# lambdaclass/simpleworks

Hardware: AMD Instinct MI355X
Metric: Marlin prove() constraints/sec at 2^20 R1CS; G1 MSM points/sec (higher is better)
Workload: dtype u32 limbs (384-bit Montgomery Fq for G1, 256-bit Fr); 1 GPU; marlin_prove: synthetic R1CS, 2^20 constraints = variables = non-zeros per matrix (|H| = |K| = 2^20), SRS + proving key device resident; per_gpu_units=1048576, multi_gpu=replicas (one proof per rank)

## Files before the change

simpleworks_amd/_lib.py:

```python
import ctypes
import json
import os

import numpy as np

_HERE = os.path.dirname(os.path.abspath(__file__))
LIB_PATH = os.environ.get("SWM_LIB_PATH") or os.path.join(_HERE, "libswmarlin.so")

_u64p = ctypes.POINTER(ctypes.c_uint64)
_u32p = ctypes.POINTER(ctypes.c_uint32)
_vp = ctypes.c_void_p
_sz = ctypes.c_size_t
_int = ctypes.c_int

ABI = {
    "swm_version": (_int, []),
    "swm_strerror": (ctypes.c_char_p, [_int]),
    "swm_init": (_int, [_int, ctypes.POINTER(_vp)]),
    "swm_destroy": (None, [_vp]),
    "swm_last_error": (ctypes.c_char_p, [_vp]),
    "swm_set_stream": (_int, [_vp, _vp]),
    "swm_set_msm_sharding": (_int, [_vp, ctypes.c_uint, ctypes.c_uint, _vp, _vp]),
    "swm_rccl_unique_id": (_int, [ctypes.c_void_p]),
    "swm_rccl_init": (_int, [_vp, ctypes.c_void_p, ctypes.c_uint, ctypes.c_uint]),
# ... 1192 lines not shown
        jac = np.zeros((n, 18), dtype=np.uint64) if backmap else None
        self._check(self.lib.swm_selftest_p28(self.h, self.P28_OPS[op], _p64(a) if a is not None else None,
                                              _p64(b) if b is not None else None, _p32(flags) if flags is not None else None,
                                              _p64(out), _p64(jac) if backmap else None, _p32(status), n), "swm_selftest_p28")
        return out, status[:n], jac

    def _poly(self, op, data, n, m, z, pieces, out):
        zz = np.ascontiguousarray(z if z is not None else np.zeros(4), dtype=np.uint64).reshape(4)
        pc = np.ascontiguousarray(pieces if pieces is not None else np.zeros(2), dtype=np.uint64).reshape(-1)
        self._check(self.lib.swm_selftest_poly(self.h, op, data.ctypes.data, n, m, _p64(zz), _p64(pc), pc.size // 2,
                                               out.ctypes.data if out is not None else None), "swm_selftest_poly")

    def selftest_suffix_recurrence(self, a_mont, m, z_mont):
        a = np.ascontiguousarray(a_mont, dtype=np.uint64).reshape(-1, 4).copy()
        self._poly(0, a, a.shape[0], m, z_mont, None, None)
        return a

    def selftest_div_linear(self, p_mont, z_mont):
        p = np.ascontiguousarray(p_mont, dtype=np.uint64).reshape(-1, 4)
        out = np.zeros_like(p)
        self._poly(1, p, p.shape[0], 0, z_mont, None, out)
        return out

    def selftest_poly_eval(self, p_mont, z_mont):
        p = np.ascontiguousarray(p_mont, dtype=np.uint64).reshape(-1, 4)
        out = np.zeros(4, dtype=np.uint64)
        self._poly(2, p, p.shape[0], 0, z_mont, None, out)
        return out

    def selftest_poly_eval_many(self, buf_mont, pieces, z_mont):
        buf = np.ascontiguousarray(buf_mont, dtype=np.uint64).reshape(-1, 4)
        pc = np.asarray(pieces, dtype=np.uint64).reshape(-1, 2)
        out = np.zeros((pc.shape[0], 4), dtype=np.uint64)
        self._poly(3, buf, buf.shape[0], 0, z_mont, pc, out)
        return out

    def selftest_ntt_from(self, src_mont, log_n, inverse=False, coset=False):
        src = np.ascontiguousarray(src_mont, dtype=np.uint64).reshape(-1, 4).copy()
        out = np.zeros((1 << log_n, 4), dtype=np.uint64)
        self._poly(4 + int(bool(inverse)) + 2 * int(bool(coset)), src, src.shape[0], log_n, None, None, out)
        return out, src

    def selftest_ntt_cosets(self, coeffs_mont, log_n, ks):
        src = np.ascontiguousarray(coeffs_mont, dtype=np.uint64).reshape(-1, 4).copy()
        kk = np.ascontiguousarray(ks, dtype=np.uint64).reshape(-1)
        out = np.zeros((kk.size << log_n, 4), dtype=np.uint64)
# ... 56 lines not shown
```

simpleworks_amd/csrc/devops.cuh:

```cuda
#pragma once
#include <chrono>
#include <exception>
#include <functional>
#include <utility>
#include <atomic>
#include "context.h"
#include "ff.cuh"
#include "fill.cuh"
#include "fr29.cuh"
#include "host/chacha.h"
#include "host/marlin_types.h"

namespace swm {

int ntt_run(swm_ctx* ctx, void* d_data, unsigned log_n, int inverse, int coset);
int ntt_run_from(swm_ctx* ctx, void* d_data, unsigned log_n, int inverse, int coset, const void* first_src, size_t src_len);
int ntt_cosets_fwd(swm_ctx* ctx, const void* coeffs, size_t len, unsigned log_n, const unsigned* ks, unsigned ncos, void* out);
int ntt_cosets_inv(swm_ctx* ctx, void* data, unsigned log_n, unsigned ncos);
int ntt_sharded_run(swm_ctx* ctx, void* d_local, unsigned log_n, int inverse, int blocks_in);
struct SpmvPlanHost {
    uint64_t nnz = 0, max_row = 0;
    std::vector<uint32_t> chunks, lrows;
};
struct SpmvPlan {
// ... 51 lines not shown
            }
        }
        p = nullptr;
    }
    void zero() { hip_check(ctx, zero_fill_async(p, n * sizeof(T), ctx->stream), "memset"); }
    void upload(const T* h, size_t count) {
        hip_check(ctx, hipMemcpyAsync(p, h, count * sizeof(T), hipMemcpyHostToDevice, ctx->stream), "h2d");
        hip_check(ctx, hipStreamSynchronize(ctx->stream), "sync");
    }
    std::vector<T> download(size_t off, size_t count) const {
        std::vector<T> h(count);
        hip_check(ctx, hipMemcpyAsync(h.data(), p + off, count * sizeof(T), hipMemcpyDeviceToHost, ctx->stream), "d2h");
        hip_check(ctx, hipStreamSynchronize(ctx->stream), "sync");
        return h;
    }
};
typedef DBuf<Fr> DVec;

inline DVec dv_zeros(swm_ctx* ctx, size_t n) {
    DVec v(ctx, n);
    v.zero();
    return v;
}
inline DVec dv_copy_padded(swm_ctx* ctx, const Fr* src, size_t len, size_t n) {
    DVec v(ctx, n);
    if (len > n) len = n;
    if (len) hip_check(ctx, hipMemcpyAsync(v.p, src, len * sizeof(Fr), hipMemcpyDeviceToDevice, ctx->stream), "d2d");
    if (n > len) hip_check(ctx, zero_fill_async(v.p + len, (n - len) * sizeof(Fr), ctx->stream), "memset");
    return v;
}

static __global__ void swm_proof_begin() {}

template <class F>
static __global__ void __launch_bounds__(256) ew_kernel(size_t n, F f) {
    SWM_LIGHT_KERNEL();
    for (size_t i = blockIdx.x * (size_t)blockDim.x + threadIdx.x; i < n; i += (size_t)gridDim.x * blockDim.x) f(i);
}
template <class F>
inline void ew(swm_ctx* ctx, const char* name, size_t n, F f) {
    if (n == 0) return;
    unsigned grid = (unsigned)std::min<size_t>((n + 255) / 256, 256 * 32);
    prof_begin(ctx, name);
    hipLaunchKernelGGL(ew_kernel<F>, dim3(grid), dim3(256), 0, ctx->stream, n, f);
    prof_end(ctx);
    hip_check(ctx, hipGetLastError(), name);
}

struct PowTable {
    const Fr* lo;
    const Fr* hi;
    __device__ __forceinline__ Fr at(uint64_t e) const {
// ... 109 lines not shown
static __global__ void __launch_bounds__(256) rec_tile_total29(const Fr* __restrict__ a, size_t n, RecConsts rc,
                                                               const Fr* __restrict__ zlow ,
                                                               Fr* __restrict__ totals) {
    SWM_LIGHT_KERNEL();
    __shared__ Fr sm[256];
    const size_t base = (size_t)blockIdx.x * RT_TILE;
    const unsigned t = threadIdx.x;
    const Fr29 z256 = fr29_unpack(rc.z256);
    Fr29 acc = fr29_zero();
#pragma unroll 1
    for (int j = RT_PER - 1; j >= 0; j--) {
        size_t k = base + (size_t)j * 256 + t;
        acc = fr29_mul_fenced(acc, z256);
        if (k < n) acc = fr29_add(acc, fr29_unpack(a[k]));
    }
    sm[t] = fr29_pack(fr29_canonical(fr29_mul_fenced(acc, fr29_unpack(zlow[t])), true));
    __syncthreads();
    for (unsigned s = 128; s > 0; s >>= 1) {
        if (t < s) sm[t] = fp_add(sm[t], sm[t + s]);
        __syncthreads();
    }
    if (t == 0) totals[blockIdx.x] = fp_mul(sm[0], rc.zpow[0]);
}
static __global__ void __launch_bounds__(256) rec_tile_scan29(Fr* __restrict__ a, size_t n, RecConsts rc,
                                                              const Fr* __restrict__ tile_true , size_t ntiles) {
    SWM_LIGHT_KERNEL();
    extern __shared__ __align__(16) unsigned char smem_raw[];
    Fr* tile = reinterpret_cast<Fr*>(smem_raw);
    Fr* hs = tile + RT_TILE + 256;
    const size_t b = blockIdx.x, base = b * RT_TILE;
    const unsigned t = threadIdx.x;
#pragma unroll
    for (int j = 0; j < RT_PER; j++) {
        unsigned e = j * 256 + t;
        size_t k = base + e;
        tile[rt_pad(e)] = k < n ? a[k] : fp_zero<Fr>();
    }
    __syncthreads();
    Fr29 loc[RT_PER];
    {
        const Fr29 z1 = fr29_unpack(rc.zpow[1]);
        Fr29 acc = fr29_zero();
#pragma unroll
        for (int i = RT_PER - 1; i >= 0; i--) {
            acc = fr29_add(fr29_unpack(tile[rt_pad(t * RT_PER + i)]), fr29_mul_fenced(acc, z1));
            loc[i] = acc;
        }
        hs[t] = fr29_pack(fr29_below_2r(acc));
    }
    if (t == 0) hs[256] = b + 1 < ntiles ? tile_true[b + 1] : fp_zero<Fr>();
    __syncthreads();
#pragma unroll 1
    for (int k = 0; k < 9; k++) {
        unsigned d = 1u << k;
        Fr v = hs[t];
        bool has = t + d <= 256;
        Fr o = has ? hs[t + d] : fp_zero<Fr>();
        __syncthreads();
        if (has) hs[t] = fr29_pack(fr29_below_2r(fr29_add(fr29_unpack(v), fr29_mul_fenced(fr29_unpack(o), fr29_unpack(rc.zstep[k])))));
        __syncthreads();
    }
    const Fr29 carry = fr29_unpack(hs[t + 1]);
#pragma unroll
    for (int i = 0; i < RT_PER; i++) {
        const Fr29 v = fr29_add(loc[i], fr29_mul_fenced(carry, fr29_unpack(rc.zpow[RT_PER - i])));
        tile[rt_pad(t * RT_PER + i)] = fr29_pack(fr29_cond_sub(fr29_cond_sub(fr29_cond_sub(fr29_normalize(v), Fr29Consts::P2), Fr29Consts::P2), Fr29Consts::P));
    }
    __syncthreads();
#pragma unroll
    for (int j = 0; j < RT_PER; j++) {
        unsigned e = j * 256 + t;
        size_t k = base + e;
        if (k < n) a[k] = tile[rt_pad(e)];
    }
}

inline void suffix_recurrence(swm_ctx* ctx, Fr* a, size_t n, size_t m, const Fr& z);
inline void suffix_recurrence_tiled(swm_ctx* ctx, Fr* a, size_t n, const Fr& z) {
    size_t ntiles = (n + RT_TILE - 1) / RT_TILE;
    RecConsts rc;
    rc.zpow[0] = fp_one<Fr>();
    for (int i = 1; i <= RT_PER; i++) rc.zpow[i] = fp_mul(rc.zpow[i - 1], z);
    rc.zstep[0] = rc.zpow[RT_PER];
    for (int k = 1; k < 9; k++) rc.zstep[k] = fp_sqr(rc.zstep[k - 1]);
    DVec zlow(ctx, 256), totals(ctx, ntiles);
    rc.z256 = dv_pow256(ctx, z, zlow.p);
    RecConsts rc29;
    const Fr two5 = fp_from_u64<Fr>(32);
    for (int i = 0; i <= RT_PER; i++) rc29.zpow[i] = fp_mul(rc.zpow[i], two5);
    for (int k = 0; k < 9; k++) rc29.zstep[k] = fp_mul(rc.zstep[k], two5);
    rc29.z256 = fp_mul(rc.z256, two5);
    prof_begin(ctx, "rec_tile_total");
    hipLaunchKernelGGL(rec_tile_total29, dim3((unsigned)ntiles), dim3(256), 0, ctx->stream, (const Fr*)a, n, rc29, (const Fr*)zlow.p, totals.p);
    prof_end(ctx);
    hip_check(ctx, hipGetLastError(), "rec_tile_total");
    Fr ztile = rc.z256;
    for (int i = 0; i < 3; i++) ztile = fp_sqr(ztile);
    static_assert(RT_TILE == 2048, "tile exponent");
    suffix_recurrence(ctx, totals.p, ntiles, 1, ztile);
    size_t lds = (size_t)(RT_TILE + 256 + 257) * sizeof(Fr);
    static std::atomic<bool> attr_set[64];
    if (!attr_set[ctx->device & 63].load(std::memory_order_acquire)) {
        hip_check(ctx, hipFuncSetAttribute((const void*)rec_tile_scan29, hipFuncAttributeMaxDynamicSharedMemorySize, (int)lds), "attr");
        attr_set[ctx->device & 63].store(true, std::memory_order_release);
    }
    prof_begin(ctx, "rec_tile_scan");
    hipLaunchKernelGGL(rec_tile_scan29, dim3((unsigned)ntiles), dim3(256), lds, ctx->stream, a, n, rc29, (const Fr*)totals.p, ntiles);
    prof_end(ctx);
    hip_check(ctx, hipGetLastError(), "rec_tile_scan");
}

inline void suffix_recurrence(swm_ctx* ctx, Fr* a, size_t n, size_t m, const Fr& z) {
    if (n == 0) return;
    if (m == 1 && n >= 4 * (size_t)RT_TILE) {
        suffix_recurrence_tiled(ctx, a, n, z);
        return;
    }
    size_t rows = (n + m - 1) / m;
    if (rows <= REC_T) {
        prof_begin(ctx, "rec_serial");
        hipLaunchKernelGGL(rec_serial, dim3((unsigned)((m + 63) / 64)), dim3(64), 0, ctx->stream, a, n, m, z);
        prof_end(ctx);
        hip_check(ctx, hipGetLastError(), "rec_serial");
        return;
    }
    size_t nblk = (rows + REC_T - 1) / REC_T;
    DVec head(ctx, nblk * m);
    unsigned grid = (unsigned)((nblk * m + 255) / 256);
    prof_begin(ctx, "rec_local");
    hipLaunchKernelGGL(rec_local, dim3(grid), dim3(256), 0, ctx->stream, a, n, m, z, head.p, nblk);
    prof_end(ctx);
    hip_check(ctx, hipGetLastError(), "rec_local");
    Fr zt = z;
    for (int i = 0; i < 4; i++) zt = fp_sqr(zt);
    static_assert(REC_T == 16, "zt exponent");
    suffix_recurrence(ctx, head.p, nblk * m, m, zt);
    prof_begin(ctx, "rec_fix");
    hipLaunchKernelGGL(rec_fix, dim3(grid), dim3(256), 0, ctx->stream, a, n, m, z, head.p, nblk);
    prof_end(ctx);
    hip_check(ctx, hipGetLastError(), "rec_fix");
}

struct DivResult {
    DVec work;
};
inline DivResult div_linear(swm_ctx* ctx, const Fr* p, size_t n, const Fr& x, size_t cap = 0) {
    DivResult r;
    r.work = dv_copy_padded(ctx, p, n, std::max<size_t>({n, cap, 1}));
    if (n == 0) r.work.zero();
    suffix_recurrence(ctx, r.work.p, n, 1, x);
    return r;
}

static constexpr int EVAL_PER = 16;
static constexpr int EVAL_TILE = 256 * EVAL_PER;
static __global__ void __launch_bounds__(256) eval_chunks(const Fr* __restrict__ c, size_t n, Fr x256, const Fr* __restrict__ xpow,
                                                          Fr* __restrict__ out) {
    SWM_LIGHT_KERNEL();
    __shared__ Fr sm[256];
    const size_t base = (size_t)blockIdx.x * EVAL_TILE;
    const unsigned t = threadIdx.x;
    Fr acc = fp_zero<Fr>();
#pragma unroll 1
    for (int j = EVAL_PER - 1; j >= 0; j--) {
        size_t k = base + (size_t)j * 256 + t;
        acc = fp_mul(acc, x256);
        if (k < n) acc = fp_add(acc, c[k]);
    }
    sm[t] = fp_mul(acc, xpow[t]);
    __syncthreads();
    for (unsigned s = 128; s > 0; s >>= 1) {
        if (t < s) sm[t] = fp_add(sm[t], sm[t + s]);
// ... 472 lines not shown
```

simpleworks_amd/csrc/marlin.hip:

```cpp
#include <stdlib.h>
#include <string.h>
#include <algorithm>
#include <chrono>
#include <functional>
#include <memory>
#include <type_traits>
#include "devops.cuh"
#include "g1.cuh"
#include "host/ahp.h"

#include "msm.h"
using namespace swm;

#define LAUNCHX(ctx, name, kernel, grid, block, shmem, ...)                         \
    do {                                                                            \
        prof_begin(ctx, name);                                                      \
        hipLaunchKernelGGL(kernel, grid, block, shmem, (ctx)->stream, __VA_ARGS__); \
        prof_end(ctx);                                                              \
        hip_check(ctx, hipGetLastError(), name);                                    \
    } while (0)

#include "host/pk_codec.h"
#include "host/host_handles.h"
struct swm_srs {
// ... 934 lines not shown
    return sp;
}
DVec shard_evals(swm_ctx* ctx, const ShardPlan& sp, const Fr* coeffs, size_t n, unsigned log) {
    const size_t len = ((size_t)1 << log) / sp.SG;
    DVec loc(ctx, len);
    Fr* out = loc.p;
    const size_t s_rank = sp.rank, s_world = sp.SG;
    ew(ctx, "shard_take_cyclic", len, [=] __device__(size_t j) {
        const size_t i = s_rank + s_world * j;
        out[j] = i < n ? coeffs[i] : fp_zero<Fr>();
    });
    rc_check(ctx, ntt_sharded_run(ctx, loc.p, log, 0, 0));
    return loc;
}
void shard_gather_cyclic(swm_ctx* ctx, const Fr* loc, size_t per, unsigned lg, Fr* dst, size_t n) {
    DVec all(ctx, per << lg);
    rc_check(ctx, shard_allgather_dev(ctx, loc, per * sizeof(Fr), all.p));
    const Fr* src = all.p;
    ew(ctx, "shard_interleave", n, [=] __device__(size_t i) { dst[i] = src[(i & (((size_t)1 << lg) - 1)) * per + (i >> lg)]; });
}
void add_rho_vh(swm_ctx* ctx, Fr* poly, uint64_t H, const Fr& rho) {
    ew(ctx, "add_rho_vh", 1, [=] __device__(size_t) {
        poly[0] = fp_sub(poly[0], rho);
        poly[H] = fp_add(poly[H], rho);
    });
}
void div_vh(swm_ctx* ctx, const Fr* q, size_t part, size_t total, Fr* h, Fr* g) {
    ew(ctx, "div_vh", 3 * part, [=] __device__(size_t j) {
        Fr acc = q[j + part];
        if (j + 2 * part < total) acc = fp_add(acc, q[j + 2 * part]);
        if (j + 3 * part < total) acc = fp_add(acc, q[j + 3 * part]);
        h[j] = acc;
        if (j < part) g[j] = fp_add(q[j], acc);
    });
}
void div_vk(swm_ctx* ctx, const Fr* q, size_t part, size_t total, Fr* h) {
    ew(ctx, "div_vk", 3 * part, [=] __device__(size_t j) {
        Fr acc = fp_zero<Fr>();
        for (uint64_t i = 1; j + i * part < total; i++) acc = fp_add(acc, q[j + i * part]);
        h[j] = acc;
    });
}
#ifndef SWM_OUTER_COSETS
#define SWM_OUTER_COSETS 1
#endif
static constexpr uint64_t OUTER_COSETS_MIN_H = 16;
struct Cosets3 {
// ... 29 lines not shown
};
struct CosetsMap {
    unsigned logD;
    __host__ __device__ size_t index(size_t p) const { return ((p & (((size_t)1 << logD) - 1)) << 2) + (p >> logD); }
    __host__ __device__ size_t position(size_t i) const { return ((i & 3) << logD) + (i >> 2); }
};
template <class F>
void with_product_map(const ShardPlan& sp, bool sharded, size_t loc, bool cosets, unsigned logD, F&& f) {
    if (sharded) f(BlocksMap{loc, loc / sp.SG, sp.rank});
    else if (cosets) f(CosetsMap{logD});
    else f(DenseMap{});
}
__device__ __forceinline__ Fr round2_outer_form(const Fr& eta_a, const Fr& eta_b, const Fr& eta_c, const Fr& ra, const Fr& a,
                                                const Fr& b, const Fr& z, const Fr& t) {
    const Fr summed = fp_add(fp_add(fp_mul(eta_c, fp_mul(a, b)), fp_mul(eta_a, a)), fp_mul(eta_b, b));
    return fp_sub(fp_mul(ra, summed), fp_mul(z, t));
}
struct IndexOnB {
    const Fr *ar, *ac, *arc, *av;
    const Fr *br, *bc, *brc, *bv;
    const Fr *cr, *cc, *crc, *cv;
};
struct Round3Challenges {
    Fr alpha, beta, ab, eta_a, eta_b, eta_c, vhab;
};
__device__ __forceinline__ Fr round3_a_minus_bf(const IndexOnB& x, const Round3Challenges& c, size_t i, const Fr& f) {
    Fr da = fp_add(fp_sub(fp_sub(c.ab, fp_mul(x.ar[i], c.alpha)), fp_mul(c.beta, x.ac[i])), x.arc[i]);
    Fr db = fp_add(fp_sub(fp_sub(c.ab, fp_mul(x.br[i], c.alpha)), fp_mul(c.beta, x.bc[i])), x.brc[i]);
    Fr dc = fp_add(fp_sub(fp_sub(c.ab, fp_mul(x.cr[i], c.alpha)), fp_mul(c.beta, x.cc[i])), x.crc[i]);
    Fr dbc = fp_mul(db, dc);
    Fr t = fp_add(fp_add(fp_mul(fp_mul(c.eta_a, x.av[i]), dbc), fp_mul(fp_mul(fp_mul(c.eta_b, x.bv[i]), da), dc)),
                  fp_mul(fp_mul(fp_mul(c.eta_c, x.cv[i]), da), db));
    Fr a_val = fp_mul(c.vhab, t);
    Fr b_val = fp_mul(da, dbc);
    return fp_sub(a_val, fp_mul(b_val, f));
}
struct ProveState {
    ChaChaRng& zk;
    PhaseTrace& tr;
    const ProveShape shape;
    const ShardPlan sp;
    const uint64_t H, K, X, Bsz, M;
    const unsigned logM;
    const size_t nvars, ninst;
    const size_t mask_len;
    const HDomain dh;
    const std::vector<Fr> public_input;
    FiatShamirRng fs;
    VerifierState st;
    Fr rho_w, rho_a, rho_b;
    int lane = 0;
    LPoly P_w, P_za, P_zb, P_mask, P_t, P_g1, P_h1, P_g2, P_h2;
    LPoly idx_polys[12];
    std::map<std::string, LPoly*> polys;
    CommitJob j1[4], j2[3], j3[2];
    std::vector<Commitment> comms1 = std::vector<Commitment>(4), comms2 = std::vector<Commitment>(3),
                            comms3 = std::vector<Commitment>(2);
    bool mask_late = false;
    unsigned mask_pieces = 1;
    AsyncMsm mask_part[2];
    bool ra_closed_form = false;
    bool cosets = false;
    LcSet lcs;
    DVec mask, z, za_evals, zb_evals, za_loc, zb_loc, x_poly, x_evals, w_poly, za_poly, zb_poly, e_za, e_zb, e_z;
    DVec r_alpha_evals, e_ra, t_poly, q1, h1, g1x, f, h2;

    ProveState(const swm_pk& pk, ChaChaRng& rng, PhaseTrace& t, ProveShape shp, const ShardPlan& plan)
        : zk(rng), tr(t), shape(std::move(shp)), sp(plan), H(pk.H), K(pk.K), X(pk.X), Bsz(pk.B), M(4 * pk.H),
          logM(pk.logH + 2), nvars(pk.info.num_variables), ninst(shape.inst.size()), mask_len(3 * pk.H), dh(pk.H),
          public_input(shape.inst.begin() + 1, shape.inst.end()) {
        fs_init(fs, pk.vk, public_input);
        for (int m = 0; m < 3; m++) {
            const DVec* v[4] = {&pk.ar[m].row, &pk.ar[m].col, &pk.ar[m].val, &pk.ar[m].row_col};
            for (int j = 0; j < 4; j++) {
                idx_polys[4 * m + j].p = v[j]->p;
                idx_polys[4 * m + j].n = K;
                polys[kIndexerPolys[4 * m + j]] = &idx_polys[4 * m + j];
            }
        }
        polys["w"] = &P_w; polys["z_a"] = &P_za; polys["z_b"] = &P_zb; polys["mask_poly"] = &P_mask;
        polys["t"] = &P_t; polys["g_1"] = &P_g1; polys["h_1"] = &P_h1; polys["g_2"] = &P_g2; polys["h_2"] = &P_h2;
    }
};

void draw_mask(swm_ctx* ctx, const swm_pk& pk, ProveState& s) {
    const uint64_t H = s.H;
    Fr* mp = s.mask.p;
// ... 92 lines not shown
                                    CommitJob* job) {
    const uint64_t H = s.H;
    const size_t sm = s.sp.sm;
    rc_check(ctx, ntt_sharded_run(ctx, loc.p, pk.logH, 1, 1));
    shard_gather_cyclic(ctx, loc.p, sm, s.sp.slog_g, poly.p, H);
    add_rho_vh(ctx, poly.p, H, rho);
    if (ctx->shard_rank == 0) {
        Fr* lp = loc.p;
        const size_t top = sm;
        ew(ctx, "add_rho_vh", 1, [=] __device__(size_t) {
            lp[0] = fp_sub(lp[0], rho);
            lp[top] = rho;
        });
    }
    job->has_bound = false;
    job->hiding = true;
    commit_enqueue_cyclic(ctx, &s.lane, pk, loc.p, ctx->shard_rank == 0 ? sm + 1 : sm, &job->plain);
}
void round1_polys(swm_ctx* ctx, const swm_pk& pk, ProveState& s) {
    const uint64_t H = s.H, X = s.X;
    s.x_poly = DVec(ctx, X);
    s.x_poly.upload(s.shape.inst.data(), X);
    dv_ntt(ctx, s.x_poly, pk.logX, true);
    s.x_evals = dv_ntt_from(ctx, s.x_poly.p, X, pk.logH, false);
    const uint64_t ratio = H / X;
    const size_t nwit = s.shape.nwit, ninst = s.ninst;
    s.w_poly = dv_zeros(ctx, H + 1);
    {
        Fr* out = s.w_poly.p;
        const Fr* zz = s.z.p;
        const Fr* xe = s.x_evals.p;
        ew(ctx, "w_evals", H, [=] __device__(size_t k) {
            Fr v = fp_zero<Fr>();
            if (k % ratio != 0) {
                size_t wi = k - k / ratio - 1;
                Fr wv = wi < nwit ? zz[ninst + wi] : fp_zero<Fr>();
                v = fp_sub(wv, xe[k]);
            }
            out[k] = v;
        });
    }
    rc_check(ctx, ntt_run(ctx, s.w_poly.p, pk.logH, 1, 0));
    add_rho_vh(ctx, s.w_poly.p, H, s.rho_w);
    suffix_recurrence(ctx, s.w_poly.p, H + 1, X, fr_one());
    s.P_w.p = s.w_poly.p + X;
    s.P_w.n = H + 1 - X;
    s.P_w.hiding = true;
    pc_commit_begin(ctx, pk, &s.lane, s.P_w.p, s.P_w.n, false, 0, true, &s.j1[0]);
    s.za_poly = dv_zeros(ctx, H + 1);
    s.zb_poly = dv_zeros(ctx, H + 1);
    s.P_za.p = s.za_poly.p; s.P_za.n = H + 1; s.P_za.hiding = true;
    s.P_zb.p = s.zb_poly.p; s.P_zb.n = H + 1; s.P_zb.hiding = true;
    if (s.sp.r1) {
        sharded_interpolate_and_commit(ctx, pk, s, s.za_loc, s.rho_a, s.za_poly, &s.j1[1]);
        sharded_interpolate_and_commit(ctx, pk, s, s.zb_loc, s.rho_b, s.zb_poly, &s.j1[2]);
    } else {
        rc_check(ctx, ntt_run_from(ctx, s.za_poly.p, pk.logH, 1, 0, s.za_evals.p, H));
        add_rho_vh(ctx, s.za_poly.p, H, s.rho_a);
        rc_check(ctx, ntt_run_from(ctx, s.zb_poly.p, pk.logH, 1, 0, s.zb_evals.p, H));
        add_rho_vh(ctx, s.zb_poly.p, H, s.rho_b);
        pc_commit_begin(ctx, pk, &s.lane, s.P_za.p, s.P_za.n, false, 0, true, &s.j1[1]);
        pc_commit_begin(ctx, pk, &s.lane, s.P_zb.p, s.P_zb.n, false, 0, true, &s.j1[2]);
    }
}

DVec on_round2_layout(swm_ctx* ctx, const ProveState& s, const Fr* coeffs, size_t n) {
    if (s.sp.r2) return shard_evals(ctx, s.sp, coeffs, n, s.logM);
    if (!s.cosets) return dv_ntt_from(ctx, coeffs, n, s.logM, false);
    static const unsigned ks[2] = {1, 2};
    DVec v(ctx, 2 * s.H);
    rc_check(ctx, ntt_cosets_fwd(ctx, coeffs, n, s.dh.log, ks, 2, v.p));
    return v;
}
void round2_prework(swm_ctx* ctx, ProveState& s) {
    const uint64_t H = s.H, X = s.X;
    s.cosets = SWM_OUTER_COSETS && !s.sp.r1 && !s.sp.r2 && H >= OUTER_COSETS_MIN_H;
    s.e_za = on_round2_layout(ctx, s, s.za_poly.p, H + 1);
    s.e_zb = on_round2_layout(ctx, s, s.zb_poly.p, H + 1);
    DVec z_poly = dv_zeros(ctx, H + 1);
    Fr* out = z_poly.p;
    const Fr* wc = s.P_w.p;
    const size_t w_len = s.P_w.n;
    const Fr* xp = s.x_poly.p;
    ew(ctx, "z_poly", H + 1, [=] __device__(size_t i) {
        Fr v = fp_zero<Fr>();
        if (i >= X && i - X < w_len) v = wc[i - X];
        if (i < w_len) v = fp_sub(v, wc[i]);
        if (i < X) v = fp_add(v, xp[i]);
        out[i] = v;
    });
    s.e_z = on_round2_layout(ctx, s, z_poly.p, H + 1);
}

void round1_commitments(swm_ctx* ctx, const swm_pk& pk, ProveState& s) {
    pc_commit_blind(pk, &s.j1[0], &s.zk, &s.P_w.rand);
    pc_commit_blind(pk, &s.j1[1], &s.zk, &s.P_za.rand);
    pc_commit_blind(pk, &s.j1[2], &s.zk, &s.P_zb.rand);
    pc_commit_blind(pk, &s.j1[3], nullptr, &s.P_mask.rand);
    if (s.mask_pieces > 1) {
        Fr c0 = s.mask.download(0, 1)[0];
        Fr c0s = fp_to_std(c0);
        G1XYZZ extra = g1_mul_limbs(pk.vk.vk.g, c0s.v, 8);
// ... 44 lines not shown
    if (s.sp.r2) r_alpha_on_h(ctx, pk, s);
}

void round2_t(swm_ctx* ctx, const swm_pk& pk, ProveState& s) {
    const uint64_t H = s.H, X = s.X;
    const size_t nvars = s.nvars;
    const Fr eta_a = s.st.eta_a, eta_b = s.st.eta_b, eta_c = s.st.eta_c;
    s.t_poly = dv_zeros(ctx, H);
    {
        DVec ta(ctx, nvars), tb(ctx, nvars), tc(ctx, nvars);
        const Fr* ra = s.r_alpha_evals.p;
        rc_check(ctx, spmv_run(ctx, pk.at.rowptr.p, pk.at.col.p, pk.at.val.p, ra, ta.p, nvars, &pk.at.plan));
        rc_check(ctx, spmv_run(ctx, pk.bt.rowptr.p, pk.bt.col.p, pk.bt.val.p, ra, tb.p, nvars, &pk.bt.plan));
        rc_check(ctx, spmv_run(ctx, pk.ct.rowptr.p, pk.ct.col.p, pk.ct.val.p, ra, tc.p, nvars, &pk.ct.plan));
        Fr* out = s.t_poly.p;
        const Fr *pa = ta.p, *pb = tb.p, *pc = tc.p;
        ew(ctx, "t_evals", nvars, [=] __device__(size_t c) {
            Fr v = fp_add(fp_add(fp_mul(eta_a, pa[c]), fp_mul(eta_b, pb[c])), fp_mul(eta_c, pc[c]));
            out[reindex_by_subdomain(H, X, c)] = v;
        });
        if (s.cosets) {
            s.q1 = DVec(ctx, 3 * H);
            Fr* q = s.q1.p;
            const Fr *rh = s.r_alpha_evals.p, *za = s.za_evals.p, *zb = s.zb_evals.p, *th = s.t_poly.p, *zz = s.z.p, *xe = s.x_evals.p;
            const uint64_t ratio = H / X;
            const size_t nwit = s.shape.nwit, ninst = s.ninst;
            ew(ctx, "round2_pointwise_h", H, [=] __device__(size_t k) {
                Fr zk = xe[k];
                if (k % ratio != 0) {
                    const size_t wi = k - k / ratio - 1;
                    zk = wi < nwit ? zz[ninst + wi] : fp_zero<Fr>();
                }
                q[k] = round2_outer_form(eta_a, eta_b, eta_c, rh[k], za[k], zb[k], zk, th[k]);
            });
        }
        dv_ntt(ctx, s.t_poly, pk.logH, true);
    }
    s.tr.tick("r2: t polynomial enqueued");
    s.P_t.p = s.t_poly.p;
    s.P_t.n = H;
    pc_commit_begin(ctx, pk, &s.lane, s.P_t.p, s.P_t.n, false, 0, false, &s.j2[0]);
}

void round2_q1(swm_ctx* ctx, const swm_pk& pk, ProveState& s) {
    const uint64_t H = s.H, M = s.M;
    const size_t Mloc = s.sp.Mloc;
    const Fr eta_a = s.st.eta_a, eta_b = s.st.eta_b, eta_c = s.st.eta_c;
    const size_t off = s.cosets ? H : 0, n = s.cosets ? 2 * H : Mloc;
    if (!s.cosets) s.q1 = DVec(ctx, Mloc);
    const Fr* mp = s.mask.p;
    {
        const Fr* pra = s.e_ra.p + off;
// ... 91 lines not shown
        }
        rc_check(ctx, batch_inverse_run(ctx, inv.p, 3 * K));
        Fr* out = s.f.p;
        const Fr *ia = inv.p, *ib = inv.p + K, *ic = inv.p + 2 * K;
        const Fr *va = pk.ar[0].val_K.p, *vb = pk.ar[1].val_K.p, *vc = pk.ar[2].val_K.p;
        if (f_cosets) {
            f_K = DVec(ctx, K);
            out = f_K.p;
        }
        ew(ctx, "round3_f_K", K, [=] __device__(size_t i) {
            Fr t = fp_add(fp_add(fp_mul(fp_mul(eta_a, va[i]), ia[i]), fp_mul(fp_mul(eta_b, vb[i]), ib[i])),
                          fp_mul(fp_mul(eta_c, vc[i]), ic[i]));
            out[i] = fp_mul(vhab, t);
        });
        if (f_cosets) rc_check(ctx, ntt_run_from(ctx, s.f.p, pk.logK, 1, 0, f_K.p, K));
        else dv_ntt(ctx, s.f, pk.logK, true);
    }
    s.P_g2.p = s.f.p + 1; s.P_g2.n = K - 1; s.P_g2.has_bound = true; s.P_g2.bound = K - 2;
    pc_commit_begin(ctx, pk, &s.lane, s.P_g2.p, s.P_g2.n, true, K - 2, false, &s.j3[0]);
    s.h2 = DVec(ctx, 3 * K);
    const IndexOnB ix{pk.ar[0].row_B.p, pk.ar[0].col_B.p, pk.ar[0].row_col_B.p, pk.ar[0].val_B.p,
                      pk.ar[1].row_B.p, pk.ar[1].col_B.p, pk.ar[1].row_col_B.p, pk.ar[1].val_B.p,
                      pk.ar[2].row_B.p, pk.ar[2].col_B.p, pk.ar[2].row_col_B.p, pk.ar[2].val_B.p};
    const Round3Challenges ch{alpha, beta, fp_mul(beta, alpha), eta_a, eta_b, eta_c, vhab};
    const size_t Bloc = s.sp.r3 ? Bsz / s.sp.SG : Bsz;
    with_product_map(s.sp, s.sp.r3, Bloc, f_cosets, pk.logK, [&](auto map) {
        constexpr bool blocks = std::is_same_v<decltype(map), BlocksMap>, cosets = std::is_same_v<decltype(map), CosetsMap>;
        DVec e_f;
        if constexpr (blocks) {
            e_f = shard_evals(ctx, s.sp, s.f.p, K, pk.logB);
        } else if constexpr (cosets) {
            static const unsigned ks[3] = {1, 2, 3};
            e_f = DVec(ctx, 3 * K);
            rc_check(ctx, ntt_cosets_fwd(ctx, s.f.p, K, pk.logK, ks, 3, e_f.p));
        } else {
            e_f = dv_ntt_from(ctx, s.f.p, K, pk.logB, false);
        }
        DVec ab(ctx, Bloc);
        Fr* out = ab.p;
        const Fr *pf = e_f.p, *fk = f_K.p;
        ew(ctx, "round3_pointwise_B", Bloc, [=] __device__(size_t p) {
            if constexpr (cosets) {
                const size_t at = map.position(p);
                out[p] = round3_a_minus_bf(ix, ch, p, at < K ? fk[at] : pf[at - K]);
            } else {
                out[p] = round3_a_minus_bf(ix, ch, map.index(p), pf[p]);
            }
        });
        if constexpr (blocks) {
            const size_t Kl = K / s.sp.SG;
            rc_check(ctx, ntt_sharded_run(ctx, ab.p, pk.logB, 1, 1));
            DVec loc(ctx, 3 * Kl);
            div_vk(ctx, ab.p, Kl, Bloc, loc.p);
            shard_gather_cyclic(ctx, loc.p, 3 * Kl, s.sp.slog_g, s.h2.p, 3 * K);
        } else {
            dv_ntt(ctx, ab, pk.logB, true);
            div_vk(ctx, ab.p, K, Bsz, s.h2.p);
        }
    });
    s.P_h2.p = s.h2.p;
    s.P_h2.n = 3 * K >= 3 ? 3 * K - 3 : 0;
}

std::vector<Fr> evaluations(swm_ctx* ctx, const swm_pk& pk, ProveState& s) {
    std::map<std::pair<std::string, bool>, Fr> eval_cache;
    {
        std::vector<std::pair<std::string, bool>> want;
        for (const char* l : {"z_b", "t", "g_1", "mask_poly", "z_a", "w", "h_1"}) want.push_back({l, false});
        for (int i = 0; i < 12; i++) want.push_back({kIndexerPolys[i], true});
// ... 56 lines not shown
}

#ifndef SWM_OPEN_FOLD
#define SWM_OPEN_FOLD 1
#endif
__global__ void __launch_bounds__(256) open_fold_shifted(Fr* __restrict__ wq, const Fr* __restrict__ sq, size_t n, Fr k) {
    SWM_LIGHT_KERNEL();
    for (size_t t = blockIdx.x * (size_t)blockDim.x + threadIdx.x; t < n; t += (size_t)gridDim.x * blockDim.x)
        wq[t] = fp_add(wq[t], fp_mul(sq[t], k));
}
std::vector<PcProof> open_combinations(swm_ctx* ctx, const swm_pk& pk, ProveState& s, const Fr& xi) {
    struct ShiftedTerm {
        LPoly* lp;
        Fr ch;
    };
    static constexpr int MAX_COMBINE = 24;
    struct CombineTerms {
        const Fr* src[MAX_COMBINE];
        size_t len[MAX_COMBINE];
        Fr k[MAX_COMBINE];
    };
    struct PointOpen {
        Fr point;
        DVec comb;
        DivResult wq;
        std::vector<DivResult> sq;
        AsyncMsm wjob;
        std::vector<AsyncMsm> sjobs;
        AsyncMsm folded_slot;
        bool folded = false;
        HPoly r_comb, shifted_r, shifted_r_witness;
        std::vector<ShiftedTerm> shifted_terms;
    };
    const char* points[2] = {"beta", "gamma"};
    PointOpen po[2];
    for (int pi = 0; pi < 2; pi++) {
        const char* pl = points[pi];
        PointOpen& o = po[pi];
        o.point = pi == 0 ? s.st.beta : s.st.gamma;
        const Fr point = o.point;
        std::vector<std::string> labels;
        for (auto& q : kQuerySet)
            if (std::string(q.point) == pl) labels.push_back(q.label);
        std::sort(labels.begin(), labels.end());
        size_t plen = 0;
        for (auto& l : labels)
            for (auto& t : s.lcs.at(l))
                if (!t.second.empty()) plen = std::max(plen, s.polys.at(t.second)->n);
        o.comb = DVec(ctx, plen ? plen : 1);
        CombineTerms cterms;
        int nterms = 0;
        Fr ch = fr_one();
        for (auto& l : labels) {
            const LcTerms& terms = s.lcs.at(l);
            bool single_bounded = false;
            for (auto& t : terms) {
                if (t.second.empty()) continue;
                LPoly* lp = s.polys.at(t.second);
                if (terms.size() == 1 && lp->has_bound) single_bounded = true;
                else if (lp->has_bound) throw MarlinError(SWM_ERR_INTERNAL, "EquationHasDegreeBounds");
                Fr k = fp_mul(ch, t.first);
                if (nterms >= MAX_COMBINE) throw MarlinError(SWM_ERR_INTERNAL, "too many terms in an opening");
                cterms.src[nterms] = lp->p;
                cterms.len[nterms] = lp->n;
                cterms.k[nterms] = k;
                nterms++;
                hp_add_scaled(o.r_comb, lp->rand.rand, k);
            }
            ch = fp_mul(ch, xi);
            if (single_bounded) {
                LPoly* lp = s.polys.at(terms[0].second);
                o.shifted_terms.push_back({lp, ch});
                hp_add_scaled(o.shifted_r, lp->rand.shifted_rand, ch);
                if (!hp_is_zero(lp->rand.shifted_rand)) hp_add_scaled(o.shifted_r_witness, hp_div_linear(lp->rand.shifted_rand, point), ch);
                ch = fp_mul(ch, xi);
            }
        }
        {
            Fr* out = o.comb.p;
            const int nt = nterms;
            ew(ctx, "open_combine", plen, [=] __device__(size_t i) {
                Fr acc = fp_zero<Fr>();
                for (int j = 0; j < nt; j++)
                    if (i < cterms.len[j]) acc = fp_add(acc, fp_mul(cterms.k[j], cterms.src[j][i]));
                out[i] = acc;
            });
        }
        s.tr.tick(pi == 0 ? "open beta: combination enqueued" : "open gamma: combination enqueued");
        size_t wn = plen ? plen - 1 : 0;
        std::vector<bool> folded(o.shifted_terms.size(), false);
        for (size_t i = 0; i < o.shifted_terms.size(); i++) {
            const LPoly* lp = o.shifted_terms[i].lp;
            const size_t off = pk.srs_max_degree - lp->bound, qn = lp->n ? lp->n - 1 : 0;
            folded[i] = SWM_OPEN_FOLD && qn && pk.in_powers(off, qn);
            if (folded[i]) wn = std::max(wn, off + qn);
        }
        o.wq = div_linear(ctx, o.comb.p, plen, point, wn + 1);
        s.tr.tick("  witness quotient enqueued");
        const bool fold_any = std::find(folded.begin(), folded.end(), true) != folded.end();
        if (!fold_any) {
            commit_enqueue(ctx, &s.lane, pk, 0, o.wq.work.p + 1, wn, &o.wjob);
            s.tr.tick("  witness commitment enqueued");
        }
        o.sq.resize(o.shifted_terms.size());
        o.sjobs.reserve(o.shifted_terms.size());
        for (size_t i = 0; i < o.shifted_terms.size(); i++) {
            auto& stt = o.shifted_terms[i];
            o.sq[i] = div_linear(ctx, stt.lp->p, stt.lp->n, point);
            Fr k = stt.ch;
            Fr* q = o.sq[i].work.p;
            const size_t off = pk.srs_max_degree - stt.lp->bound, qn = stt.lp->n ? stt.lp->n - 1 : 0;
            if (folded[i]) {
                const unsigned grid = (unsigned)std::min<size_t>((qn + 255) / 256, 256 * 32);
                LAUNCHX(ctx, "open_fold_shifted", open_fold_shifted, dim3(grid), dim3(256), 0, o.wq.work.p + 1 + off, q + 1, qn, k);
                s.tr.tick("  shifted quotient folded");
                continue;
            }
            ew(ctx, "open_scale", qn, [=] __device__(size_t t) { q[t + 1] = fp_mul(q[t + 1], k); });
            s.tr.tick("  shifted quotient enqueued");
            o.sjobs.emplace_back();
// ... 637 lines not shown
        unsigned ks[4];
        for (size_t c = 0; c < npieces; c++) ks[c] = (unsigned)pieces[c];
        DVec t(ctx, npieces << m);
        rc_check(ctx, ntt_cosets_fwd(ctx, a.p, n, (unsigned)m, ks, (unsigned)npieces, t.p));
        std::vector<Fr> h = t.download(0, t.n);
        memcpy(out, h.data(), t.n * sizeof(Fr));
        return;
    }
    if (op == 10) {
        const size_t N = (size_t)1 << m;
        rc_check(ctx, ntt_cosets_inv(ctx, a.p, (unsigned)m, 3));
        DVec t(ctx, 3 * N);
        const Fr* u = a.p;
        Fr* o = t.p;
        const Fr iota = HDomain(4).gen, half = fr_half();
        ew(ctx, "cosets3_solve", N, [=] __device__(size_t j) {
            const Cosets3 c = cosets3_solve(u[j], u[j + N], u[j + 2 * N], iota, half);
            o[j] = c.p0;
            o[j + N] = c.p1;
            o[j + 2 * N] = c.p2;
        });
        std::vector<Fr> h = t.download(0, t.n);
        memcpy(out, h.data(), t.n * sizeof(Fr));
        return;
    }
    if (op == 0) {
        suffix_recurrence(ctx, a.p, n, m, zz);
        std::vector<Fr> h = a.download(0, n);
        if (n) memcpy(data, h.data(), n * sizeof(Fr));
    } else if (op == 1) {
        DivResult r = div_linear(ctx, a.p, n, zz);
        std::vector<Fr> h = r.work.download(0, n);
        if (n) memcpy(out, h.data(), n * sizeof(Fr));
    } else if (op == 2) {
        const Fr v = poly_eval(ctx, a.p, n, zz);
        memcpy(out, v.v, sizeof(Fr));
    } else if (op == 3) {
        for (size_t i = 0; i < npieces; i++)
            if (pieces[2 * i] > n || pieces[2 * i + 1] > n - pieces[2 * i]) throw MarlinError(SWM_ERR_INVALID_ARG, "piece out of range");
        DVec res(ctx, npieces);
        std::vector<EvalItem> items;
        for (size_t i = 0; i < npieces; i++) items.push_back({a.p + pieces[2 * i], (size_t)pieces[2 * i + 1], res.p + i});
        EvalPoint ep = eval_point(ctx, zz);
        poly_eval_many(ctx, items, ep);
        std::vector<Fr> h = res.download(0, npieces);
        if (npieces) memcpy(out, h.data(), npieces * sizeof(Fr));
    } else {
        DVec t = dv_ntt_from(ctx, a.p, n, (unsigned)m, ((op - 4) & 1) != 0, ((op - 4) & 2) != 0);
        std::vector<Fr> h = t.download(0, t.n);
        memcpy(out, h.data(), t.n * sizeof(Fr));
        std::vector<Fr> s = a.download(0, n);
        if (n) memcpy(data, s.data(), n * sizeof(Fr));
    }
}
int swm_selftest_poly(swm_ctx* ctx, int op, void* data, size_t n, size_t m, const uint64_t z[4], const uint64_t* pieces,
                      size_t npieces, void* out) {
    if (!ctx || op < 0 || op > 10 || (n && !data)) return SWM_ERR_INVALID_ARG;
    if ((op >= 1 && op <= 3 && !z) || (op == 0 && (!z || m == 0)) || (op != 0 && !out) || (op == 3 && npieces && !pieces))
        return SWM_ERR_INVALID_ARG;
    if (op >= 4 && op <= 7 && (m < 1 || m > 28 || n > ((size_t)1 << m))) return SWM_ERR_INVALID_ARG;
    if (op == 9) {
        if (m < 1 || m > 26 || n > ((size_t)2 << m) || npieces < 1 || npieces > 4 || !pieces) return SWM_ERR_INVALID_ARG;
        for (size_t c = 0; c < npieces; c++)
            if (pieces[c] > 3) return SWM_ERR_INVALID_ARG;
    }
    if (op == 10 && (m < 1 || m > 26 || n != ((size_t)3 << m))) return SWM_ERR_INVALID_ARG;
    SWM_ON_DEVICE(ctx);
    SWM_GUARD(ctx, selftest_poly_impl(ctx, op, data, n, m, z, pieces, npieces, out));
}
static void selftest_spmv_plan_impl(swm_ctx* ctx, const uint32_t* rowptr, const uint32_t* col, const uint64_t* val, size_t rows,
                                    const uint64_t* z, size_t z_len, uint64_t* out, uint32_t* plan_counts) {
    const size_t nnz = rowptr[rows];
    HostCsr m;
    m.rowptr.assign(rowptr, rowptr + rows + 1);
    m.col.assign(col, col + nnz);
    m.val.resize(nnz);
    if (nnz) memcpy(m.val.data(), val, nnz * sizeof(Fr));
    DevCsr d = upload_csr(ctx, m);
    DVec dz(ctx, z_len), o(ctx, rows);
    dz.upload((const Fr*)z, z_len);
// ... 103 lines not shown
```

Baseline: 22.90 million constraints/s.

## Fuse copy-pad into recurrence and drop redundant buffers in Marlin prover

```diff
diff --git a/simpleworks_amd/_lib.py b/simpleworks_amd/_lib.py
--- a/simpleworks_amd/_lib.py
+++ b/simpleworks_amd/_lib.py
@@ -1238,6 +1238,12 @@
         self._poly(1, p, p.shape[0], 0, z_mont, None, out)
         return out
 
+    def selftest_div_linear_from(self, p_mont, z_mont, cap):
+        p = np.ascontiguousarray(p_mont, dtype=np.uint64).reshape(-1, 4).copy()
+        out = np.zeros((cap, 4), dtype=np.uint64)
+        self._poly(11, p, p.shape[0], cap, z_mont, None, out)
+        return out, p
+
     def selftest_poly_eval(self, p_mont, z_mont):
         p = np.ascontiguousarray(p_mont, dtype=np.uint64).reshape(-1, 4)
         out = np.zeros(4, dtype=np.uint64)
diff --git a/simpleworks_amd/csrc/devops.cuh b/simpleworks_amd/csrc/devops.cuh
--- a/simpleworks_amd/csrc/devops.cuh
+++ b/simpleworks_amd/csrc/devops.cuh
@@ -97,12 +97,27 @@
     v.zero();
     return v;
 }
-inline DVec dv_copy_padded(swm_ctx* ctx, const Fr* src, size_t len, size_t n) {
-    DVec v(ctx, n);
-    if (len > n) len = n;
-    if (len) hip_check(ctx, hipMemcpyAsync(v.p, src, len * sizeof(Fr), hipMemcpyDeviceToDevice, ctx->stream), "d2d");
-    if (n > len) hip_check(ctx, zero_fill_async(v.p + len, (n - len) * sizeof(Fr), ctx->stream), "memset");
-    return v;
+static __global__ void __launch_bounds__(256) copy_pad_kernel(uint4* __restrict__ dst, const uint4* __restrict__ src, size_t len,
+                                                              size_t n) {
+    SWM_LIGHT_KERNEL();
+    const size_t stride = (size_t)gridDim.x * blockDim.x;
+    for (size_t i = (size_t)blockIdx.x * blockDim.x + threadIdx.x; i < n; i += stride)
+        dst[i] = i < len ? src[i] : make_uint4(0u, 0u, 0u, 0u);
+}
+inline void dv_copy_pad_into(swm_ctx* ctx, Fr* dst, const Fr* src, size_t len, size_t n) {
+    if (n == 0) return;
+    if ((((uintptr_t)dst | (uintptr_t)src) & 15) != 0) {
+        if (len) hip_check(ctx, hipMemcpyAsync(dst, src, len * sizeof(Fr), hipMemcpyDeviceToDevice, ctx->stream), "d2d");
+        if (n > len) hip_check(ctx, zero_fill_async(dst + len, (n - len) * sizeof(Fr), ctx->stream), "memset");
+        return;
+    }
+    static_assert(sizeof(Fr) == 2 * sizeof(uint4), "element = two 16-byte pieces");
+    const unsigned grid = (unsigned)std::min<size_t>((2 * n + 255) / 256, 2048);
+    prof_begin(ctx, "copy_pad");
+    hipLaunchKernelGGL(copy_pad_kernel, dim3(grid), dim3(256), 0, ctx->stream, reinterpret_cast<uint4*>(dst),
+                       reinterpret_cast<const uint4*>(src), 2 * len, 2 * n);
+    prof_end(ctx);
+    hip_check(ctx, hipGetLastError(), "copy_pad");
 }
 
 static __global__ void swm_proof_begin() {}
@@ -258,7 +273,7 @@
     }
     if (t == 0) totals[blockIdx.x] = fp_mul(sm[0], rc.zpow[0]);
 }
-static __global__ void __launch_bounds__(256) rec_tile_scan29(Fr* __restrict__ a, size_t n, RecConsts rc,
+static __global__ void __launch_bounds__(256) rec_tile_scan29(const Fr* src, Fr* dst, size_t n, size_t cap, RecConsts rc,
                                                               const Fr* __restrict__ tile_true , size_t ntiles) {
     SWM_LIGHT_KERNEL();
     extern __shared__ __align__(16) unsigned char smem_raw[];
@@ -266,11 +281,19 @@
     Fr* hs = tile + RT_TILE + 256;
     const size_t b = blockIdx.x, base = b * RT_TILE;
     const unsigned t = threadIdx.x;
+    if (b >= ntiles) {
+#pragma unroll
+        for (int j = 0; j < RT_PER; j++) {
+            size_t k = base + j * 256 + t;
+            if (k < cap) dst[k] = fp_zero<Fr>();
+        }
+        return;
+    }
 #pragma unroll
     for (int j = 0; j < RT_PER; j++) {
         unsigned e = j * 256 + t;
         size_t k = base + e;
-        tile[rt_pad(e)] = k < n ? a[k] : fp_zero<Fr>();
+        tile[rt_pad(e)] = k < n ? src[k] : fp_zero<Fr>();
     }
     __syncthreads();
     Fr29 loc[RT_PER];
@@ -307,12 +330,13 @@
     for (int j = 0; j < RT_PER; j++) {
         unsigned e = j * 256 + t;
         size_t k = base + e;
-        if (k < n) a[k] = tile[rt_pad(e)];
+        if (k < n) dst[k] = tile[rt_pad(e)];
+        else if (k < cap) dst[k] = fp_zero<Fr>();
     }
 }
 
 inline void suffix_recurrence(swm_ctx* ctx, Fr* a, size_t n, size_t m, const Fr& z);
-inline void suffix_recurrence_tiled(swm_ctx* ctx, Fr* a, size_t n, const Fr& z) {
+inline void suffix_recurrence_tiled(swm_ctx* ctx, const Fr* src, Fr* dst, size_t n, size_t cap, const Fr& z) {
     size_t ntiles = (n + RT_TILE - 1) / RT_TILE;
     RecConsts rc;
     rc.zpow[0] = fp_one<Fr>();
@@ -327,7 +351,7 @@
     for (int k = 0; k < 9; k++) rc29.zstep[k] = fp_mul(rc.zstep[k], two5);
     rc29.z256 = fp_mul(rc.z256, two5);
     prof_begin(ctx, "rec_tile_total");
-    hipLaunchKernelGGL(rec_tile_total29, dim3((unsigned)ntiles), dim3(256), 0, ctx->stream, (const Fr*)a, n, rc29, (const Fr*)zlow.p, totals.p);
+    hipLaunchKernelGGL(rec_tile_total29, dim3((unsigned)ntiles), dim3(256), 0, ctx->stream, src, n, rc29, (const Fr*)zlow.p, totals.p);
     prof_end(ctx);
     hip_check(ctx, hipGetLastError(), "rec_tile_total");
     Fr ztile = rc.z256;
@@ -341,7 +365,9 @@
         attr_set[ctx->device & 63].store(true, std::memory_order_release);
     }
     prof_begin(ctx, "rec_tile_scan");
-    hipLaunchKernelGGL(rec_tile_scan29, dim3((unsigned)ntiles), dim3(256), lds, ctx->stream, a, n, rc29, (const Fr*)totals.p, ntiles);
+    const size_t grid = (std::max(n, cap) + RT_TILE - 1) / RT_TILE;
+    hipLaunchKernelGGL(rec_tile_scan29, dim3((unsigned)grid), dim3(256), lds, ctx->stream, src, dst, n, std::max(n, cap), rc29,
+                       (const Fr*)totals.p, ntiles);
     prof_end(ctx);
     hip_check(ctx, hipGetLastError(), "rec_tile_scan");
 }
@@ -349,7 +375,7 @@
 inline void suffix_recurrence(swm_ctx* ctx, Fr* a, size_t n, size_t m, const Fr& z) {
     if (n == 0) return;
     if (m == 1 && n >= 4 * (size_t)RT_TILE) {
-        suffix_recurrence_tiled(ctx, a, n, z);
+        suffix_recurrence_tiled(ctx, a, a, n, n, z);
         return;
     }
     size_t rows = (n + m - 1) / m;
@@ -380,10 +406,25 @@
 struct DivResult {
     DVec work;
 };
+inline void suffix_recurrence_from(swm_ctx* ctx, const Fr* src, Fr* dst, size_t n, size_t cap, const Fr& z) {
+    if (cap < n) cap = n;
+    if (n >= 4 * (size_t)RT_TILE) {
+        suffix_recurrence_tiled(ctx, src, dst, n, cap, z);
+        return;
+    }
+    dv_copy_pad_into(ctx, dst, src, n, cap);
+    suffix_recurrence(ctx, dst, n, 1, z);
+}
 inline DivResult div_linear(swm_ctx* ctx, const Fr* p, size_t n, const Fr& x, size_t cap = 0) {
     DivResult r;
-    r.work = dv_copy_padded(ctx, p, n, std::max<size_t>({n, cap, 1}));
-    if (n == 0) r.work.zero();
+    const size_t len = std::max<size_t>({n, cap, 1});
+    r.work = DVec(ctx, len);
+    suffix_recurrence_from(ctx, p, r.work.p, n, len, x);
+    return r;
+}
+inline DivResult div_linear_in_place(swm_ctx* ctx, DVec&& work, size_t n, const Fr& x) {
+    DivResult r;
+    r.work = std::move(work);
     suffix_recurrence(ctx, r.work.p, n, 1, x);
     return r;
 }
diff --git a/simpleworks_amd/csrc/marlin.hip b/simpleworks_amd/csrc/marlin.hip
--- a/simpleworks_amd/csrc/marlin.hip
+++ b/simpleworks_amd/csrc/marlin.hip
@@ -980,7 +980,7 @@
 void add_rho_vh(swm_ctx* ctx, Fr* poly, uint64_t H, const Fr& rho) {
     ew(ctx, "add_rho_vh", 1, [=] __device__(size_t) {
         poly[0] = fp_sub(poly[0], rho);
-        poly[H] = fp_add(poly[H], rho);
+        poly[H] = rho;
     });
 }
 void div_vh(swm_ctx* ctx, const Fr* q, size_t part, size_t total, Fr* h, Fr* g) {
@@ -1056,16 +1056,15 @@
     const Fr *cr, *cc, *crc, *cv;
 };
 struct Round3Challenges {
-    Fr alpha, beta, ab, eta_a, eta_b, eta_c, vhab;
+    Fr alpha, beta, ab, ve_a, ve_b, ve_c;
 };
 __device__ __forceinline__ Fr round3_a_minus_bf(const IndexOnB& x, const Round3Challenges& c, size_t i, const Fr& f) {
     Fr da = fp_add(fp_sub(fp_sub(c.ab, fp_mul(x.ar[i], c.alpha)), fp_mul(c.beta, x.ac[i])), x.arc[i]);
     Fr db = fp_add(fp_sub(fp_sub(c.ab, fp_mul(x.br[i], c.alpha)), fp_mul(c.beta, x.bc[i])), x.brc[i]);
     Fr dc = fp_add(fp_sub(fp_sub(c.ab, fp_mul(x.cr[i], c.alpha)), fp_mul(c.beta, x.cc[i])), x.crc[i]);
     Fr dbc = fp_mul(db, dc);
-    Fr t = fp_add(fp_add(fp_mul(fp_mul(c.eta_a, x.av[i]), dbc), fp_mul(fp_mul(fp_mul(c.eta_b, x.bv[i]), da), dc)),
-                  fp_mul(fp_mul(fp_mul(c.eta_c, x.cv[i]), da), db));
-    Fr a_val = fp_mul(c.vhab, t);
+    Fr ua = fp_mul(c.ve_a, x.av[i]), ub = fp_mul(c.ve_b, x.bv[i]), uc = fp_mul(c.ve_c, x.cv[i]);
+    Fr a_val = fp_add(fp_mul(ua, dbc), fp_mul(da, fp_add(fp_mul(ub, dc), fp_mul(uc, db))));
     Fr b_val = fp_mul(da, dbc);
     return fp_sub(a_val, fp_mul(b_val, f));
 }
@@ -1096,7 +1095,7 @@
     bool ra_closed_form = false;
     bool cosets = false;
     LcSet lcs;
-    DVec mask, z, za_evals, zb_evals, za_loc, zb_loc, x_poly, x_evals, w_poly, za_poly, zb_poly, e_za, e_zb, e_z;
+    DVec mask, z, za_evals, zb_evals, za_loc, zb_loc, x_poly, w_poly, za_poly, zb_poly, e_za, e_zb, e_z;
     DVec r_alpha_evals, e_ra, t_poly, q1, h1, g1x, f, h2;
 
     ProveState(const swm_pk& pk, ChaChaRng& rng, PhaseTrace& t, ProveShape shp, const ShardPlan& plan)
@@ -1235,33 +1234,37 @@
     s.x_poly = DVec(ctx, X);
     s.x_poly.upload(s.shape.inst.data(), X);
     dv_ntt(ctx, s.x_poly, pk.logX, true);
-    s.x_evals = dv_ntt_from(ctx, s.x_poly.p, X, pk.logH, false);
     const uint64_t ratio = H / X;
     const size_t nwit = s.shape.nwit, ninst = s.ninst;
-    s.w_poly = dv_zeros(ctx, H + 1);
+    s.w_poly = DVec(ctx, H + 1);
     {
         Fr* out = s.w_poly.p;
         const Fr* zz = s.z.p;
-        const Fr* xe = s.x_evals.p;
         ew(ctx, "w_evals", H, [=] __device__(size_t k) {
-            Fr v = fp_zero<Fr>();
-            if (k % ratio != 0) {
+            Fr v;
+            if (k % ratio == 0) {
+                v = zz[k / ratio];
+            } else {
                 size_t wi = k - k / ratio - 1;
-                Fr wv = wi < nwit ? zz[ninst + wi] : fp_zero<Fr>();
-                v = fp_sub(wv, xe[k]);
+                v = wi < nwit ? zz[ninst + wi] : fp_zero<Fr>();
             }
             out[k] = v;
         });
     }
     rc_check(ctx, ntt_run(ctx, s.w_poly.p, pk.logH, 1, 0));
+    {
+        Fr* out = s.w_poly.p;
+        const Fr* xp = s.x_poly.p;
+        ew(ctx, "w_sub_x", X, [=] __device__(size_t i) { out[i] = fp_sub(out[i], xp[i]); });
+    }
     add_rho_vh(ctx, s.w_poly.p, H, s.rho_w);
     suffix_recurrence(ctx, s.w_poly.p, H + 1, X, fr_one());
     s.P_w.p = s.w_poly.p + X;
     s.P_w.n = H + 1 - X;
     s.P_w.hiding = true;
     pc_commit_begin(ctx, pk, &s.lane, s.P_w.p, s.P_w.n, false, 0, true, &s.j1[0]);
-    s.za_poly = dv_zeros(ctx, H + 1);
-    s.zb_poly = dv_zeros(ctx, H + 1);
+    s.za_poly = DVec(ctx, H + 1);
+    s.zb_poly = DVec(ctx, H + 1);
     s.P_za.p = s.za_poly.p; s.P_za.n = H + 1; s.P_za.hiding = true;
     s.P_zb.p = s.zb_poly.p; s.P_zb.n = H + 1; s.P_zb.hiding = true;
     if (s.sp.r1) {
@@ -1290,7 +1293,7 @@
     s.cosets = SWM_OUTER_COSETS && !s.sp.r1 && !s.sp.r2 && H >= OUTER_COSETS_MIN_H;
     s.e_za = on_round2_layout(ctx, s, s.za_poly.p, H + 1);
     s.e_zb = on_round2_layout(ctx, s, s.zb_poly.p, H + 1);
-    DVec z_poly = dv_zeros(ctx, H + 1);
+    DVec z_poly(ctx, H + 1);
     Fr* out = z_poly.p;
     const Fr* wc = s.P_w.p;
     const size_t w_len = s.P_w.n;
@@ -1381,12 +1384,14 @@
         if (s.cosets) {
             s.q1 = DVec(ctx, 3 * H);
             Fr* q = s.q1.p;
-            const Fr *rh = s.r_alpha_evals.p, *za = s.za_evals.p, *zb = s.zb_evals.p, *th = s.t_poly.p, *zz = s.z.p, *xe = s.x_evals.p;
+            const Fr *rh = s.r_alpha_evals.p, *za = s.za_evals.p, *zb = s.zb_evals.p, *th = s.t_poly.p, *zz = s.z.p;
             const uint64_t ratio = H / X;
             const size_t nwit = s.shape.nwit, ninst = s.ninst;
             ew(ctx, "round2_pointwise_h", H, [=] __device__(size_t k) {
-                Fr zk = xe[k];
-                if (k % ratio != 0) {
+                Fr zk;
+                if (k % ratio == 0) {
+                    zk = zz[k / ratio];
+                } else {
                     const size_t wi = k - k / ratio - 1;
                     zk = wi < nwit ? zz[ninst + wi] : fp_zero<Fr>();
                 }
@@ -1524,7 +1529,7 @@
     const IndexOnB ix{pk.ar[0].row_B.p, pk.ar[0].col_B.p, pk.ar[0].row_col_B.p, pk.ar[0].val_B.p,
                       pk.ar[1].row_B.p, pk.ar[1].col_B.p, pk.ar[1].row_col_B.p, pk.ar[1].val_B.p,
                       pk.ar[2].row_B.p, pk.ar[2].col_B.p, pk.ar[2].row_col_B.p, pk.ar[2].val_B.p};
-    const Round3Challenges ch{alpha, beta, fp_mul(beta, alpha), eta_a, eta_b, eta_c, vhab};
+    const Round3Challenges ch{alpha, beta, fp_mul(beta, alpha), fp_mul(vhab, eta_a), fp_mul(vhab, eta_b), fp_mul(vhab, eta_c)};
     const size_t Bloc = s.sp.r3 ? Bsz / s.sp.SG : Bsz;
     with_product_map(s.sp, s.sp.r3, Bloc, f_cosets, pk.logK, [&](auto map) {
         constexpr bool blocks = std::is_same_v<decltype(map), BlocksMap>, cosets = std::is_same_v<decltype(map), CosetsMap>;
@@ -1540,13 +1545,14 @@
         }
         DVec ab(ctx, Bloc);
         Fr* out = ab.p;
-        const Fr *pf = e_f.p, *fk = f_K.p;
+        const bool on_K_every_4th = Bsz == 4 * K;
+        const Fr* pf = e_f.p;
         ew(ctx, "round3_pointwise_B", Bloc, [=] __device__(size_t p) {
             if constexpr (cosets) {
-                const size_t at = map.position(p);
-                out[p] = round3_a_minus_bf(ix, ch, p, at < K ? fk[at] : pf[at - K]);
+                out[p] = (p & 3) == 0 ? fp_zero<Fr>() : round3_a_minus_bf(ix, ch, p, pf[map.position(p) - K]);
             } else {
-                out[p] = round3_a_minus_bf(ix, ch, map.index(p), pf[p]);
+                const size_t i = map.index(p);
+                out[p] = on_K_every_4th && (i & 3) == 0 ? fp_zero<Fr>() : round3_a_minus_bf(ix, ch, i, pf[p]);
             }
         });
         if constexpr (blocks) {
@@ -1649,7 +1655,6 @@
     };
     struct PointOpen {
         Fr point;
-        DVec comb;
         DivResult wq;
         std::vector<DivResult> sq;
         AsyncMsm wjob;
@@ -1674,7 +1679,6 @@
         for (auto& l : labels)
             for (auto& t : s.lcs.at(l))
                 if (!t.second.empty()) plen = std::max(plen, s.polys.at(t.second)->n);
-        o.comb = DVec(ctx, plen ? plen : 1);
         CombineTerms cterms;
         int nterms = 0;
         Fr ch = fr_one();
@@ -1703,17 +1707,6 @@
                 ch = fp_mul(ch, xi);
             }
         }
-        {
-            Fr* out = o.comb.p;
-            const int nt = nterms;
-            ew(ctx, "open_combine", plen, [=] __device__(size_t i) {
-                Fr acc = fp_zero<Fr>();
-                for (int j = 0; j < nt; j++)
-                    if (i < cterms.len[j]) acc = fp_add(acc, fp_mul(cterms.k[j], cterms.src[j][i]));
-                out[i] = acc;
-            });
-        }
-        s.tr.tick(pi == 0 ? "open beta: combination enqueued" : "open gamma: combination enqueued");
         size_t wn = plen ? plen - 1 : 0;
         std::vector<bool> folded(o.shifted_terms.size(), false);
         for (size_t i = 0; i < o.shifted_terms.size(); i++) {
@@ -1722,7 +1715,19 @@
             folded[i] = SWM_OPEN_FOLD && qn && pk.in_powers(off, qn);
             if (folded[i]) wn = std::max(wn, off + qn);
         }
-        o.wq = div_linear(ctx, o.comb.p, plen, point, wn + 1);
+        {
+            DVec work(ctx, std::max<size_t>(plen, wn + 1));
+            Fr* out = work.p;
+            const int nt = nterms;
+            ew(ctx, "open_combine", work.n, [=] __device__(size_t i) {
+                Fr acc = fp_zero<Fr>();
+                for (int j = 0; j < nt; j++)
+                    if (i < cterms.len[j]) acc = fp_add(acc, fp_mul(cterms.k[j], cterms.src[j][i]));
+                out[i] = acc;
+            });
+            s.tr.tick(pi == 0 ? "open beta: combination enqueued" : "open gamma: combination enqueued");
+            o.wq = div_linear_in_place(ctx, std::move(work), plen, point);
+        }
         s.tr.tick("  witness quotient enqueued");
         const bool fold_any = std::find(folded.begin(), folded.end(), true) != folded.end();
         if (!fold_any) {
@@ -2406,6 +2411,17 @@
         });
         std::vector<Fr> h = t.download(0, t.n);
         memcpy(out, h.data(), t.n * sizeof(Fr));
+        return;
+    }
+    if (op == 11) {
+        const size_t cap = std::max<size_t>(m, 1);
+        DVec dst(ctx, cap);
+        hip_check(ctx, hipMemsetAsync(dst.p, 0xFF, cap * sizeof(Fr), ctx->stream), "memset");
+        suffix_recurrence_from(ctx, a.p, dst.p, n, cap, zz);
+        std::vector<Fr> h = dst.download(0, cap);
+        memcpy(out, h.data(), cap * sizeof(Fr));
+        std::vector<Fr> src = a.download(0, n);
+        if (n) memcpy(data, src.data(), n * sizeof(Fr));
         return;
     }
     if (op == 0) {
@@ -2439,7 +2455,8 @@
 }
 int swm_selftest_poly(swm_ctx* ctx, int op, void* data, size_t n, size_t m, const uint64_t z[4], const uint64_t* pieces,
                       size_t npieces, void* out) {
-    if (!ctx || op < 0 || op > 10 || (n && !data)) return SWM_ERR_INVALID_ARG;
+    if (!ctx || op < 0 || op > 11 || (n && !data)) return SWM_ERR_INVALID_ARG;
+    if (op == 11 && (!z || m < n || m < 1)) return SWM_ERR_INVALID_ARG;
     if ((op >= 1 && op <= 3 && !z) || (op == 0 && (!z || m == 0)) || (op != 0 && !out) || (op == 3 && npieces && !pieces))
         return SWM_ERR_INVALID_ARG;
     if (op >= 4 && op <= 7 && (m < 1 || m > 28 || n > ((size_t)1 << m))) return SWM_ERR_INVALID_ARG;
```

New measurement: 23.13 million constraints/s, median of 6. 1.0% higher.
